# PaddlePaddle/MetaGym

Hardware: AMD Instinct MI355X
Metric: env-steps/sec (whole node) at 2^16 parallel envs; 1/2/4/8-GPU scaling (higher is better)
Workload: dtype f32/f64 mixed (reference choreography)

## Files before the change

metagym_amd/csrc/quadrotor.hip:

```cpp
#include <cstdlib>

#include "mg_common.h"
#include "mg_philox.h"

namespace {

#ifndef MG_QUAD_BLOCK
#define MG_QUAD_BLOCK 256
#endif
constexpr int BLOCK = MG_QUAD_BLOCK;
constexpr int WAVES_PER_BLOCK = BLOCK / mg::WAVE;
constexpr int OBS_DIM = 16;

struct QuadK {
    float phi32, phi_over_ra32, inv_jm32, mm32, prec32, ct0_32, ct1_32;
    float quality32, dt32, zoff32, healthy32, fail_range_sq32;
    float lm[4];
    float pc[12];
    float iinv[9];
    float df[9], dm[9];
    float cog[3];
    double prec, half_dt2, half_dt, ct2, quality, inv_quality;
    double min_v, max_v, fail_velocity, fail_w, healthy, xoff, yoff;
    int quality_recip_exact;
    int times, nt, task;
    int auto_reset;
    float init_v_base[3], init_w_base[3];
    double init_v_noisy, init_w_noisy;
    uint64_t seed, env_id_base;
    const int32_t *map;
    int map_h, map_w;
    const float *vtargets;
    int obs_dim;
};

struct Lane {
    float p[3];
    double v[3];
    double w[3];
    float pw[4];
    float R[9];
    double Rd[9];
    float Ri[9];
    double nv, nw;
    float power;
};


__device__ __forceinline__ double dot_row_f32f64(const float *row, const double *x) {
    return fma((double)row[2], x[2], fma((double)row[0], x[0], (double)row[1] * x[1]));
}

__device__ __forceinline__ void mv_f32f64(const float *M, const double *x, double *y) {
#pragma unroll
    for (int r = 0; r < 3; ++r) y[r] = dot_row_f32f64(&M[3 * r], x);
}

__device__ __forceinline__ void mv_f32(const float *M, const float *x, float *y) {
#pragma unroll
    for (int r = 0; r < 2; ++r) y[r] = (M[3 * r] * x[0] + M[3 * r + 1] * x[1]) + M[3 * r + 2] * x[2];
    y[2] = fmaf(M[8], x[2], fmaf(M[6], x[0], M[7] * x[1]));
}

__device__ __forceinline__ void mm_f32(const float *A, const float *B, float *C) {
#pragma unroll
    for (int r = 0; r < 3; ++r)
#pragma unroll
        for (int c = 0; c < 3; ++c)
            C[3 * r + c] = fmaf(A[3 * r + 2], B[6 + c], fmaf(A[3 * r + 1], B[3 + c], A[3 * r] * B[c]));
}

__device__ __forceinline__ void cross_f32(const float *a, const float *b, float *c) {
    float t0 = a[1] * b[2], t1 = a[2] * b[1];
    float t2 = a[2] * b[0], t3 = a[0] * b[2];
    float t4 = a[0] * b[1], t5 = a[1] * b[0];
    c[0] = t0 - t1;
    c[1] = t2 - t3;
    c[2] = t4 - t5;
}

__device__ __forceinline__ double norm3(const double *x) {
    return sqrt(fma(x[2], x[2], fma(x[1], x[1], x[0] * x[0])));
}
__device__ __forceinline__ float sumsq3(const float *x) {
    const float p0 = x[0] * x[0], p1 = x[1] * x[1], p2 = x[2] * x[2];
    return (float)(((double)p0 + (double)p1) + (double)p2);
}

__device__ __forceinline__ void inv3(const float *Af, float *Ainv, double *A) {
#pragma unroll
    for (int i = 0; i < 9; ++i) A[i] = (double)Af[i];
    const double c00 = fma(A[4], A[8], -(A[5] * A[7]));
    const double c01 = fma(A[5], A[6], -(A[3] * A[8]));
    const double c02 = fma(A[3], A[7], -(A[4] * A[6]));
    const double det = fma(A[2], c02, fma(A[1], c01, A[0] * c00));
    const double r = 1.0 / det;
    Ainv[0] = (float)(c00 * r);
    Ainv[3] = (float)(c01 * r);
    Ainv[6] = (float)(c02 * r);
    Ainv[1] = (float)(fma(A[2], A[7], -(A[1] * A[8])) * r);
    Ainv[4] = (float)(fma(A[0], A[8], -(A[2] * A[6])) * r);
    Ainv[7] = (float)(fma(A[1], A[6], -(A[0] * A[7])) * r);
    Ainv[2] = (float)(fma(A[1], A[5], -(A[2] * A[4])) * r);
    Ainv[5] = (float)(fma(A[2], A[3], -(A[0] * A[5])) * r);
    Ainv[8] = (float)(fma(A[0], A[4], -(A[1] * A[3])) * r);
}

template <bool SIMPLE, bool RECIP = false, bool XF = false>
__device__ __forceinline__ void substep(const QuadK &k, Lane &s, const float *eff32, bool want_power) {
    static_assert(!XF || SIMPLE, "the X frame is a SIMPLE configuration");
    float prop_force_z = 0.0f;
    float prop_torque[3] = {0.0f, 0.0f, 0.0f};
    float me[4], pp[4];

    const double bvz = dot_row_f32f64(&s.Ri[6], s.v);
    double xcz[4];
    if (XF) {
        const double c = (double)k.pc[1];
        const double A = s.w[0] * c, B = s.w[1] * c;
        xcz[0] = A - B;
        xcz[1] = A + B;
        xcz[2] = B - A;
        xcz[3] = (-A) - B;
    }

#pragma unroll
    for (int i = 0; i < 4; ++i) {
        const float e32 = eff32[i];
        float phi_w = k.phi32 * s.pw[i];
        me[i] = k.phi_over_ra32 * (e32 - phi_w);
        if (want_power) pp[i] = fabsf(me[i] / k.phi32 * e32);
        float d_prop_w = k.inv_jm32 * (me[i] - k.mm32);
        float w_m = s.pw[i] + k.prec32 * d_prop_w;
        const float *pc = &k.pc[3 * i];
        double cz = XF ? xcz[i] : s.w[0] * (double)pc[1] - s.w[1] * (double)pc[0];
        double v_1 = bvz + cz * (double)(XF ? k.lm[0] : k.lm[i]);
        float t0 = (k.ct0_32 * w_m) * w_m;
        double t1 = (double)(k.ct1_32 * w_m) * v_1;
        double thrust = (double)t0 + t1;
        if (!SIMPLE) {
            double sign = v_1 > 0 ? 1.0 : -1.0;
            thrust = thrust + ((k.ct2 * v_1) * v_1) * sign;
        }
        s.pw[i] = w_m;
        prop_force_z = (float)((double)prop_force_z + thrust);
        const float T = (float)thrust;
        if (XF) {
            const float Tc = T * k.pc[1];
            prop_torque[0] = (i < 2) ? prop_torque[0] + Tc : prop_torque[0] - Tc;
            prop_torque[1] = (i == 1 || i == 2) ? prop_torque[1] + Tc : prop_torque[1] - Tc;
        } else if (SIMPLE) {
            prop_torque[0] += T * pc[1];
            prop_torque[1] += (-T) * pc[0];
        } else {
            float a[3] = {-0.0f, -0.0f, -T};
            float cr[3];
            cross_f32(a, pc, cr);
            prop_torque[0] += cr[0];
            prop_torque[1] += cr[1];
            prop_torque[2] += cr[2];
        }
    }
    prop_torque[2] += ((-me[0] + me[1]) - me[2]) + me[3];

    float DfRi[9];
    double tmp[3], f_drag[3], t_drag[3];
    if (SIMPLE) {
#pragma unroll
        for (int r = 0; r < 3; ++r)
#pragma unroll
            for (int c = 0; c < 3; ++c) DfRi[3 * r + c] = k.df[4 * r] * s.Ri[3 * r + c];
    } else {
        mm_f32(k.df, s.Ri, DfRi);
    }
    mv_f32f64(DfRi, s.v, tmp);
    const double mnv = -s.nv;
#pragma unroll
    for (int c = 0; c < 3; ++c) f_drag[c] = mnv * tmp[c];
    if (SIMPLE) {
#pragma unroll
        for (int c = 0; c < 3; ++c) tmp[c] = (double)k.dm[4 * c] * s.w[c];
    } else {
        mv_f32f64(k.dm, s.w, tmp);
    }
    const double mnw = -s.nw;
#pragma unroll
    for (int c = 0; c < 3; ++c) t_drag[c] = mnw * tmp[c];

    float f_grav[3];
#pragma unroll
    for (int c = 0; c < 3; ++c) f_grav[c] = (s.Ri[3 * c + 2] * -9.8f) * k.quality32;

    double t_all[3], body_acc[3], acc[3];
    float t_grav_neg[3] = {0.0f, 0.0f, 0.0f};
    if (!SIMPLE) {
        float t_grav[3];
        cross_f32(f_grav, k.cog, t_grav);
#pragma unroll
        for (int c = 0; c < 3; ++c) t_grav_neg[c] = -t_grav[c];
    }
#pragma unroll
    for (int c = 0; c < 3; ++c) {
        const float pf = (c == 2) ? prop_force_z : 0.0f;
        double f_all = (double)(pf + f_grav[c]) + f_drag[c];
        t_all[c] = (double)(SIMPLE ? prop_torque[c] : prop_torque[c] + t_grav_neg[c]) + t_drag[c];
        body_acc[c] = (RECIP || k.quality_recip_exact) ? f_all * k.inv_quality : f_all / k.quality;
    }
#pragma unroll
    for (int r = 0; r < 3; ++r)
        acc[r] = fma(s.Rd[3 * r + 2], body_acc[2], fma(s.Rd[3 * r], body_acc[0], s.Rd[3 * r + 1] * body_acc[1]));
#pragma unroll
    for (int c = 0; c < 3; ++c)
        s.p[c] = (float)((double)s.p[c] + (s.v[c] * k.prec + k.half_dt2 * acc[c]));
#pragma unroll
    for (int c = 0; c < 3; ++c) s.v[c] = s.v[c] + k.prec * acc[c];
    if (want_power) s.power = ((pp[0] + pp[1]) + pp[2]) + pp[3];

    double alpha[3], tw[3];
    if (SIMPLE) {
#pragma unroll
        for (int c = 0; c < 3; ++c) alpha[c] = (double)k.iinv[4 * c] * t_all[c];
    } else {
        mv_f32f64(k.iinv, t_all, alpha);
    }
#pragma unroll
    for (int c = 0; c < 3; ++c) tw[c] = s.w[c] + k.half_dt * alpha[c];
    const float s01 = (float)(-tw[2]), s02 = (float)(tw[1]);
    const float s10 = (float)(tw[2]), s12 = (float)(-tw[0]);
    const float s20 = (float)(-tw[1]), s21 = (float)(tw[0]);
#pragma unroll
    for (int r = 0; r < 3; ++r) {
        const float r0 = s.R[3 * r], r1 = s.R[3 * r + 1], r2 = s.R[3 * r + 2];
        const float rs0 = fmaf(r2, s20, fmaf(r1, s10, r0 * 0.0f));
        const float rs1 = fmaf(r2, s21, fmaf(r1, 0.0f, r0 * s01));
        const float rs2 = fmaf(r2, 0.0f, fmaf(r1, s12, r0 * s02));
        s.R[3 * r] = r0 + k.prec32 * rs0;
        s.R[3 * r + 1] = r1 + k.prec32 * rs1;
        s.R[3 * r + 2] = r2 + k.prec32 * rs2;
    }
#pragma unroll
    for (int c = 0; c < 3; ++c) s.w[c] = s.w[c] + k.prec * alpha[c];
    inv3(s.R, s.Ri, s.Rd);
    s.nv = norm3(s.v);
    s.nw = norm3(s.w);
}

__device__ __forceinline__ int failure_code(const QuadK &k, const Lane &s) {
    const int c3 = (s.nw > k.fail_w) ? 3 : 0;
    const int c2 = (s.nv > k.fail_velocity) ? 2 : c3;
    return (sumsq3(s.p) > k.fail_range_sq32) ? 1 : c2;
}

__device__ __forceinline__ void observe(const QuadK &k, const Lane &s, float *obs) {
    double b_v[3];
    float b_pos[3], imu[3];
    const float g[3] = {0.0f, 0.0f, -9.8f};
    mv_f32f64(s.Ri, s.v, b_v);
    mv_f32(s.Ri, s.p, b_pos);
    mv_f32(s.Ri, g, imu);
    float roll = atan2f(s.R[7], s.R[8]);
    float pitch = atan2f(-s.R[6], sqrtf(s.R[7] * s.R[7] + s.R[8] * s.R[8]));
    float yaw = atan2f(s.R[3], s.R[0]);
    obs[0] = (float)b_v[0]; obs[1] = (float)b_v[1]; obs[2] = (float)b_v[2];
    obs[3] = b_pos[0]; obs[4] = b_pos[1]; obs[5] = b_pos[2];
    obs[6] = 0.0f + imu[0]; obs[7] = 0.0f + imu[1]; obs[8] = 0.0f + imu[2];
    obs[9] = (float)s.w[0]; obs[10] = (float)s.w[1]; obs[11] = (float)s.w[2];
    obs[12] = pitch; obs[13] = roll; obs[14] = yaw;
    obs[15] = s.p[2] + k.zoff32;
}

__device__ __forceinline__ void py_slice(long a, long b, long len, long &lo, long &hi) {
    if (a < 0) { a += len; if (a < 0) a = 0; } else if (a > len) a = len;
    if (b < 0) { b += len; if (b < 0) b = 0; } else if (b > len) b = len;
    lo = a; hi = b;
}

__device__ __forceinline__ bool collision(const QuadK &k, const double *op, const double *np_) {
    long mn[3], mx[3];
#pragma unroll
    for (int i = 0; i < 3; ++i) {
        double lo = op[i] < np_[i] ? op[i] : np_[i];
        double hi = op[i] > np_[i] ? op[i] : np_[i];
        mn[i] = (long)floor(lo);
        mx[i] = (long)ceil(hi);
    }
    int any = 0;
    if (k.map != nullptr) {
        long y0, y1, x0, x1;
        py_slice(mn[1], mx[1] + 1, k.map_h, y0, y1);
        py_slice(mn[0], mx[0] + 1, k.map_w, x0, x1);
        for (long y = y0; y < y1; ++y)
            for (long x = x0; x < x1; ++x) any |= (k.map[y * k.map_w + x] != 0);
    }
    return (mn[2] < any) || (mx[2] < any);
}

struct Lane32 {
    float p[3], v[3], w[3], pw[4], R[9], Ri[9];
};

__device__ void substep_f32state(const QuadK &k, Lane32 &s, const float *eff32) {
    float prop_force_z = 0.0f, prop_torque[3] = {0.0f, 0.0f, 0.0f}, me[4];
    const float ct2_32 = (float)k.ct2;
    for (int i = 0; i < 4; ++i) {
        const float e32 = eff32[i];
        float phi_w = k.phi32 * s.pw[i];
        me[i] = k.phi_over_ra32 * (e32 - phi_w);
        float d_prop_w = k.inv_jm32 * (me[i] - k.mm32);
        float w_m = s.pw[i] + k.prec32 * d_prop_w;
        const float *pc = &k.pc[3 * i];
        float bv[3], cr[3];
        mv_f32(s.Ri, s.v, bv);
        cross_f32(s.w, pc, cr);
        float v_1 = bv[2] + cr[2] * k.lm[i];
        float sign = v_1 > 0 ? 1.0f : -1.0f;
        float thrust = ((k.ct0_32 * w_m) * w_m + (k.ct1_32 * w_m) * v_1) + ((ct2_32 * v_1) * v_1) * sign;
        s.pw[i] = w_m;
        prop_force_z = prop_force_z + thrust;
        float a[3] = {-0.0f, -0.0f, -thrust};
        cross_f32(a, pc, cr);
        prop_torque[0] += cr[0]; prop_torque[1] += cr[1]; prop_torque[2] += cr[2];
    }
    prop_torque[2] += ((-me[0] + me[1]) - me[2]) + me[3];
    float DfRi[9], tmp[3], f_drag[3], t_drag[3];
    mm_f32(k.df, s.Ri, DfRi);
    mv_f32(DfRi, s.v, tmp);
    const float nv = -sqrtf(sumsq3(s.v));
    for (int c = 0; c < 3; ++c) f_drag[c] = nv * tmp[c];
    mv_f32(k.dm, s.w, tmp);
    const float nw = -sqrtf(sumsq3(s.w));
    for (int c = 0; c < 3; ++c) t_drag[c] = nw * tmp[c];
    const float g[3] = {0.0f, 0.0f, -9.8f};
    float f_grav[3], t_grav[3], body_acc[3], t_all[3], acc[3];
    mv_f32(s.Ri, g, f_grav);
    for (int c = 0; c < 3; ++c) f_grav[c] = f_grav[c] * k.quality32;
    cross_f32(f_grav, k.cog, t_grav);
    for (int c = 0; c < 3; ++c) {
        const float pf = (c == 2) ? prop_force_z : 0.0f;
        const float f_all = (pf + f_grav[c]) + f_drag[c];
        t_all[c] = (prop_torque[c] + (-t_grav[c])) + t_drag[c];
        body_acc[c] = f_all / k.quality32;
    }
    mv_f32(s.R, body_acc, acc);
    const float half_dt2 = (float)k.half_dt2, half_dt = (float)k.half_dt;
    for (int c = 0; c < 3; ++c) s.p[c] = s.p[c] + (s.v[c] * k.prec32 + half_dt2 * acc[c]);
    for (int c = 0; c < 3; ++c) s.v[c] = s.v[c] + k.prec32 * acc[c];
    float alpha[3], tw[3];
    mv_f32(k.iinv, t_all, alpha);
    for (int c = 0; c < 3; ++c) tw[c] = s.w[c] + half_dt * alpha[c];
    float S[9] = {0.0f, -tw[2], tw[1], tw[2], 0.0f, -tw[0], -tw[1], tw[0], 0.0f};
    float RS[9];
    mm_f32(s.R, S, RS);
    for (int c = 0; c < 9; ++c) s.R[c] = s.R[c] + k.prec32 * RS[c];
    for (int c = 0; c < 3; ++c) s.w[c] = s.w[c] + k.prec32 * alpha[c];
    double Rd[9];
    inv3(s.R, s.Ri, Rd);
}

__global__ void quadrotor_targets_kernel(QuadK k, int nt, const float *actions, float *targets) {
    if (blockIdx.x != 0 || threadIdx.x != 0) return;
    Lane32 s;
    for (int c = 0; c < 3; ++c) { s.p[c] = 0.0f; s.v[c] = 0.0f; s.w[c] = 0.0f; }
    for (int c = 0; c < 4; ++c) s.pw[c] = 0.0f;
    for (int c = 0; c < 9; ++c) { s.R[c] = (c % 4 == 0) ? 1.0f : 0.0f; s.Ri[c] = s.R[c]; }
    for (int t = 0; t < nt; ++t) {
        float eff32[4];
        for (int i = 0; i < 4; ++i) {
            double d = (double)actions[4 * t + i];
            d = d > k.max_v ? k.max_v : (d < k.min_v ? k.min_v : d);
            eff32[i] = (float)d;
        }
        for (int it = 0; it < k.times; ++it) substep_f32state(k, s, eff32);
        targets[3 * t] = s.v[0]; targets[3 * t + 1] = s.v[1]; targets[3 * t + 2] = s.v[2];
    }
}


template <typename T> __device__ __forceinline__ void st_stream(T *p, T v) { __builtin_nontemporal_store(v, p); }
typedef float v4f __attribute__((ext_vector_type(4)));
typedef uint32_t v2u __attribute__((ext_vector_type(2)));
typedef uint32_t v4u __attribute__((ext_vector_type(4)));

constexpr int AUX_NT = 2;
__device__ __forceinline__ __amdgpu_buffer_rsrc_t rsrc_of(const void *base, uint32_t bytes) {
    return __builtin_amdgcn_make_buffer_rsrc(const_cast<void *>(base), (short)0, (int)bytes, 0x00020000);
}
template <typename T> __device__ __forceinline__ T buf_ld(__amdgpu_buffer_rsrc_t r, uint32_t vo, uint32_t so) {
    if constexpr (sizeof(T) == 4) return __builtin_bit_cast(T, __builtin_amdgcn_raw_buffer_load_b32(r, vo, so, 0));
    else if constexpr (sizeof(T) == 8) return __builtin_bit_cast(T, __builtin_amdgcn_raw_buffer_load_b64(r, vo, so, 0));
    else return __builtin_bit_cast(T, __builtin_amdgcn_raw_buffer_load_b128(r, vo, so, 0));
}
template <int AUX, typename T> __device__ __forceinline__ void buf_st(T v, __amdgpu_buffer_rsrc_t r, uint32_t vo, uint32_t so) {
    if constexpr (sizeof(T) == 1) __builtin_amdgcn_raw_buffer_store_b8(__builtin_bit_cast(uint8_t, v), r, vo, so, AUX);
    else if constexpr (sizeof(T) == 4) __builtin_amdgcn_raw_buffer_store_b32(__builtin_bit_cast(uint32_t, v), r, vo, so, AUX);
    else if constexpr (sizeof(T) == 8) __builtin_amdgcn_raw_buffer_store_b64(__builtin_bit_cast(v2u, v), r, vo, so, AUX);
    else __builtin_amdgcn_raw_buffer_store_b128(__builtin_bit_cast(v4u, v), r, vo, so, AUX);
}
template <bool BUF, typename T> __device__ __forceinline__ T ld_soa(const T *a, int comps, int n, int c, int e) {
    if (!BUF) return a[(size_t)c * n + e];
    return buf_ld<T>(rsrc_of(a, (uint32_t)comps * (uint32_t)n * sizeof(T)), (uint32_t)e * sizeof(T),
                     (uint32_t)c * (uint32_t)n * sizeof(T));
}
template <bool BUF, typename T> __device__ __forceinline__ void st_soa(T *a, int comps, int n, int c, int e, T v) {
    if (!BUF) return st_stream(&a[(size_t)c * n + e], v);
    buf_st<AUX_NT>(v, rsrc_of(a, (uint32_t)comps * (uint32_t)n * sizeof(T)), (uint32_t)e * sizeof(T),
                   (uint32_t)c * (uint32_t)n * sizeof(T));
}

template <bool ROT_FIRST = false, bool BUF = false>
__device__ __forceinline__ void load_state(const mg_quadrotor_state &st, int n, int e, Lane &s, int &ct) {
    if (ROT_FIRST) {
#pragma unroll
        for (int c = 0; c < 9; ++c) s.R[c] = ld_soa<BUF>(st.rot, 9, n, c, e);
    }
    if (!ROT_FIRST) {
#pragma unroll
        for (int c = 0; c < 3; ++c) s.p[c] = ld_soa<BUF>(st.pos, 3, n, c, e);
    }
#pragma unroll
    for (int c = 0; c < 3; ++c) s.v[c] = ld_soa<BUF>(st.vel, 3, n, c, e);
#pragma unroll
    for (int c = 0; c < 3; ++c) s.w[c] = ld_soa<BUF>(st.omega, 3, n, c, e);
    if (ROT_FIRST) {
#pragma unroll
        for (int c = 0; c < 3; ++c) s.p[c] = ld_soa<BUF>(st.pos, 3, n, c, e);
    }
#pragma unroll
    for (int c = 0; c < 4; ++c) s.pw[c] = ld_soa<BUF>(st.propw, 4, n, c, e);
    if (!ROT_FIRST) {
#pragma unroll
        for (int c = 0; c < 9; ++c) s.R[c] = ld_soa<BUF>(st.rot, 9, n, c, e);
    }
    ct = ld_soa<BUF>(st.ct, 1, n, 0, e);
}

__device__ __forceinline__ void derive_lane(Lane &s) {
    inv3(s.R, s.Ri, s.Rd);
    s.nv = norm3(s.v);
    s.nw = norm3(s.w);
    s.power = 0.0f;
}

template <bool BUF = false>
__device__ __forceinline__ void load_lane(const mg_quadrotor_state &st, int n, int e, Lane &s, int &ct) {
    load_state<false, BUF>(st, n, e, s, ct);
    derive_lane(s);
}

template <bool BUF = false>
__device__ __forceinline__ void store_lane(const mg_quadrotor_state &st, int n, int e, const Lane &s, int ct) {
#pragma unroll
    for (int c = 0; c < 3; ++c) st_soa<BUF>(st.pos, 3, n, c, e, s.p[c]);
#pragma unroll
    for (int c = 0; c < 3; ++c) st_soa<BUF>(st.vel, 3, n, c, e, s.v[c]);
#pragma unroll
    for (int c = 0; c < 3; ++c) st_soa<BUF>(st.omega, 3, n, c, e, s.w[c]);
#pragma unroll
    for (int c = 0; c < 4; ++c) st_soa<BUF>(st.propw, 4, n, c, e, s.pw[c]);
#pragma unroll
    for (int c = 0; c < 9; ++c) st_soa<BUF>(st.rot, 9, n, c, e, s.R[c]);
    st_soa<BUF>(st.ct, 1, n, 0, e, ct);
}

template <bool BUF = false>
__device__ __forceinline__ void store_obs_wave(float *tile, const float *obs, float *out, int n, int e, int obs_dim) {
    if (!BUF && obs_dim != OBS_DIM) {
        if (e < n)
            for (int c = 0; c < obs_dim; ++c) out[(size_t)e * obs_dim + c] = obs[c];
        return;
    }
    const int lane = threadIdx.x & (mg::WAVE - 1);
    const int wave_base = e - lane;
    const bool full = (wave_base + mg::WAVE) <= n;
    if (full) {
#pragma unroll
        for (int c = 0; c < OBS_DIM; ++c) tile[lane * (OBS_DIM + 1) + c] = obs[c];
        __builtin_amdgcn_wave_barrier();
        float4 *dst = reinterpret_cast<float4 *>(out + (size_t)wave_base * OBS_DIM);
        const __amdgpu_buffer_rsrc_t r = rsrc_of(out, (uint32_t)n * (OBS_DIM * 4));
#pragma unroll
        for (int j = 0; j < 4; ++j) {
            const int q = j * mg::WAVE + lane;
            const int row = q >> 2, col = (q & 3) * 4;
            const float *src = &tile[row * (OBS_DIM + 1) + col];
            const v4f v{src[0], src[1], src[2], src[3]};
            if (BUF) buf_st<AUX_NT>(v, r, (uint32_t)(wave_base * OBS_DIM + 4 * lane) * 4 + j * (mg::WAVE * 16), 0);
            else st_stream(reinterpret_cast<v4f *>(dst + q), v);
        }
        __builtin_amdgcn_wave_barrier();
    } else if (e < n) {
        float4 *dst = reinterpret_cast<float4 *>(out + (size_t)e * OBS_DIM);
        const __amdgpu_buffer_rsrc_t r = rsrc_of(out, (uint32_t)n * (OBS_DIM * 4));
#pragma unroll
        for (int j = 0; j < 4; ++j) {
            const v4f v{obs[4 * j], obs[4 * j + 1], obs[4 * j + 2], obs[4 * j + 3]};
            if (BUF) buf_st<0>(v, r, (uint32_t)e * (OBS_DIM * 4) + j * 16, 0);
            else dst[j] = make_float4(v.x, v.y, v.z, v.w);
        }
    }
}

struct ResetDraw {
    double v[3], w[3], nv, nw;
};

__device__ __forceinline__ ResetDraw reset_draw(const QuadK &k, int e, uint32_t episode) {
    uint32_t r[8];
    const uint64_t gid = k.env_id_base + (uint64_t)e;
#pragma unroll
    for (int b = 0; b < 2; ++b)
        philox4x32_10((uint32_t)gid, (uint32_t)(gid >> 32), episode, (uint32_t)b, (uint32_t)k.seed,
                      (uint32_t)(k.seed >> 32), &r[4 * b]);
    const double inv32 = 1.0 / 4294967296.0;
    ResetDraw d;
#pragma unroll
    for (int c = 0; c < 3; ++c) {
        const double sv = ((r[6] >> c) & 1u) ? 1.0 : -1.0;
        const double sw = ((r[6] >> (3 + c)) & 1u) ? 1.0 : -1.0;
        d.v[c] = (double)k.init_v_base[c] + (k.init_v_noisy * ((double)r[c] * inv32)) * sv;
        d.w[c] = (double)k.init_w_base[c] + (k.init_w_noisy * ((double)r[3 + c] * inv32)) * sw;
    }
    d.nv = norm3(d.v);
    d.nw = norm3(d.w);
    return d;
}

__device__ __forceinline__ void reset_apply(Lane &s, const ResetDraw &d) {
#pragma unroll
    for (int c = 0; c < 3; ++c) {
        s.p[c] = 0.0f;
        s.v[c] = d.v[c];
        s.w[c] = d.w[c];
    }
#pragma unroll
    for (int c = 0; c < 4; ++c) s.pw[c] = 0.0f;
#pragma unroll
    for (int c = 0; c < 9; ++c) {
        s.R[c] = (c % 4 == 0) ? 1.0f : 0.0f;
        s.Ri[c] = s.R[c];
        s.Rd[c] = (double)s.R[c];
    }
    s.nv = d.nv;
    s.nw = d.nw;
    s.power = 0.0f;
}


struct StepIO {
    const float *action;
    float *obs;
    float *reward;
    double *reward64;
    uint8_t *done;
    uint8_t *failed;
};

struct KArgs { QuadK k; mg_quadrotor_state st; StepIO io; int n; int n_steps; };
typedef const __attribute__((address_space(4))) KArgs KArgsC;
__device__ __forceinline__ KArgsC *kernargs_fresh() {
    KArgsC *p = (KArgsC *)__builtin_amdgcn_kernarg_segment_ptr();
    asm volatile("" : "+s"(p));
    return p;
}

enum StepForm { STEP_GENERIC = 0, STEP_STOCK = 1, STEP_STOCK_SHADOW = 2 };
constexpr int STOCK_TIMES = 10;
#ifndef MG_QUAD_SUBSTEP_UNROLL
#define MG_QUAD_SUBSTEP_UNROLL 9
#endif

template <bool SIMPLE, int FORM, bool XF = false, bool BUF = false>
__global__ __launch_bounds__(BLOCK) void quadrotor_step_kernel(QuadK k, mg_quadrotor_state st, StepIO io,
                                                               int n, int n_steps_arg) {
    constexpr bool STOCK = FORM != STEP_GENERIC;
    constexpr bool SHADOW = FORM == STEP_STOCK_SHADOW;
    static_assert(!STOCK || SIMPLE, "the stock forms are SIMPLE");
    static_assert(STOCK || !XF, "XF is an option of the stock forms");
    static_assert(SHADOW || !BUF, "BUF is an option of STEP_STOCK_SHADOW");
    const int n_steps = SHADOW ? 1 : n_steps_arg;
    __shared__ float tiles[WAVES_PER_BLOCK][mg::WAVE * (OBS_DIM + 1)];
    const int e = blockIdx.x * BLOCK + threadIdx.x;
    const bool live = e < n;
    const int el = live ? e : n - 1;
    float *tile = tiles[threadIdx.x / mg::WAVE];

    {
        const uint32_t *ka = (const uint32_t *)__builtin_amdgcn_kernarg_segment_ptr();
        uint32_t touch = 0;
#pragma unroll
        for (int line = 0; line < (int)((sizeof(QuadK) + sizeof(mg_quadrotor_state) + sizeof(StepIO) + 8 + 63) / 64); ++line)
            touch |= ka[line * 16];
        asm volatile("" ::"s"(touch));
    }
    float4 a_next;
    Lane s;
    int ct;
    uint32_t episode = 0;
    ResetDraw rd;
    if (SHADOW) {
        episode = ld_soa<BUF>(st.episode, 1, n, 0, el);
        a_next = ld_soa<BUF>(reinterpret_cast<const float4 *>(io.action), 1, n, 0, el);
        load_state<true, BUF>(st, n, el, s, ct);
        __builtin_amdgcn_sched_barrier(0);
        rd = reset_draw(k, el, episode);
#pragma unroll
        for (int c = 0; c < 3; ++c) asm volatile("" : "+v"(rd.v[c]), "+v"(rd.w[c]));
        asm volatile("" : "+v"(rd.nv), "+v"(rd.nw));
        __builtin_amdgcn_sched_barrier(0);
        derive_lane(s);
        __builtin_amdgcn_sched_barrier(0);
    } else {
        a_next = reinterpret_cast<const float4 *>(io.action)[el];
        __builtin_amdgcn_sched_barrier(0);
        if (STOCK || k.auto_reset) episode = st.episode[el];
        load_lane(st, n, el, s, ct);
    }
    const uint32_t episode_in = episode;
    __builtin_amdgcn_s_waitcnt(0x0F70);

    for (int t = 0; t < n_steps; ++t) {
        const size_t off = (size_t)t * n;
        const float4 a = a_next;
        if (t + 1 < n_steps)
            a_next = reinterpret_cast<const float4 *>(io.action)[off + n + el];
        const float av[4] = {a.x, a.y, a.z, a.w};
        float eff32[4];
#pragma unroll
        for (int i = 0; i < 4; ++i) {
            double d = (double)av[i];
            d = d > k.max_v ? k.max_v : (d < k.min_v ? k.min_v : d);
            eff32[i] = (float)d;
        }
        ct += 1;
        const double old_pos[3] = {(double)s.p[0] + k.xoff, (double)s.p[1] + k.yoff,
                                   (double)(s.p[2] + k.zoff32)};
        int fail = 0;
        if (STOCK) {
#pragma unroll MG_QUAD_SUBSTEP_UNROLL
            for (int it = 0; it < STOCK_TIMES - 1; ++it) {
                substep<SIMPLE, true, XF>(k, s, eff32, false);
                const int code = failure_code(k, s);
                fail = fail ? fail : code;
            }
            substep<SIMPLE, true, XF>(k, s, eff32, true);
            const int code = failure_code(k, s);
            fail = fail ? fail : code;
        } else {
            for (int it = 0; it < k.times; ++it) {
                if (fail == 0) {
                    substep<SIMPLE>(k, s, eff32, it == k.times - 1);
                    fail = failure_code(k, s);
                }
            }
        }
        const KArgsC *kae = kernargs_fresh();
        const QuadK &ke = *(const QuadK *)&kae->k;
        const StepIO &ioe = *(const StepIO *)&kae->io;
        const bool vel_task = ke.task == MG_QUADROTOR_TASK_VELOCITY_CONTROL;
        const int tn_step = ct < ke.nt - 1 ? ct : ke.nt - 1;
        double reward = 0.0;
        int done = 1;
        if (fail == 0 && vel_task) {
            float bt[3];
            mv_f32(s.Ri, &ke.vtargets[3 * (ct - 1)], bt);
            double b_v[3];
            mv_f32f64(s.Ri, s.v, b_v);
            const double diff = (fabs((double)bt[0] - b_v[0]) + fabs((double)bt[1] - b_v[1])) + fabs((double)bt[2] - b_v[2]);
            const float energy = ke.dt32 * s.power;
            const double r = (ke.healthy32 < energy) ? -ke.healthy : -(double)energy;
            reward = r + (-0.001 * diff);
            done = 0;
            if (ct == ke.nt) { done = 1; ct = 0; }
        } else if (fail == 0) {
            const double new_pos[3] = {(double)s.p[0] + ke.xoff, (double)s.p[1] + ke.yoff,
                                       (double)(s.p[2] + ke.zoff32)};
            const bool hit = collision(ke, old_pos, new_pos);
            const float energy = ke.dt32 * s.power;
            double r = (ke.healthy32 < energy) ? -ke.healthy : -(double)energy;
            double task_reward = hit ? 0.0 : ke.healthy;
            if (ke.task == MG_QUADROTOR_TASK_HOVERING_CONTROL) {
                task_reward -= 1.0 * s.nv + 1.0 * s.nw;
                const float z_move = fabsf(0.0f - s.p[2]);
                if (z_move < 0.5f) task_reward += 10;
                else {
                    const float o = 0.5f - z_move;
                    task_reward += (o > -20.0f) ? (double)o : -20.0;
                }
            }
            if (ke.task == MG_QUADROTOR_TASK_HOVERING_CONTROL || ke.healthy32 < energy)
                reward = r + task_reward;
            else
                reward = (double)((float)r + (float)task_reward);
            done = 0;
            if (hit) { done = 1; ct = 0; }
            if (ct == ke.nt) { done = 1; ct = 0; }
        } else {
            ct = 0;
        }
        int tn = tn_step;
        if ((STOCK || ke.auto_reset) && done) {
            if (SHADOW) reset_apply(s, rd);
            else reset_apply(s, reset_draw(ke, el, episode));
            episode += 1;
            tn = ct < ke.nt - 1 ? ct : ke.nt - 1;
        }
        if (t + 1 < n_steps) asm volatile("" : "+v"(a_next.x), "+v"(a_next.y), "+v"(a_next.z), "+v"(a_next.w));
        if (t == n_steps - 1 && live) {
            const mg_quadrotor_state &ste = *(const mg_quadrotor_state *)&kae->st;
            store_lane<BUF>(ste, n, e, s, ct);
            if (episode != episode_in) st_soa<BUF>(ste.episode, 1, n, 0, e, episode);
        }
        __builtin_amdgcn_sched_barrier(0);
        float obs[OBS_DIM + 3];
        observe(ke, s, obs);
        if (vel_task) { obs[16] = ke.vtargets[3 * tn]; obs[17] = ke.vtargets[3 * tn + 1]; obs[18] = ke.vtargets[3 * tn + 2]; }
        store_obs_wave<BUF>(tile, obs, ioe.obs + off * ke.obs_dim, n, e, ke.obs_dim);
        if (live) {
            if (BUF) {
                if (ioe.reward) st_soa<true>(ioe.reward + off, 1, n, 0, e, (float)reward);
                if (ioe.reward64) st_soa<true>(ioe.reward64 + off, 1, n, 0, e, reward);
                st_soa<true>(ioe.done + off, 1, n, 0, e, (uint8_t)done);
                if (ioe.failed) st_soa<true>(ioe.failed + off, 1, n, 0, e, (uint8_t)fail);
            } else {
                if (ioe.reward) st_stream(&ioe.reward[off + e], (float)reward);
                if (ioe.reward64) st_stream(&ioe.reward64[off + e], reward);
                st_stream(&ioe.done[off + e], (uint8_t)done);
                if (ioe.failed) st_stream(&ioe.failed[off + e], (uint8_t)fail);
            }
        }
    }
}

__global__ __launch_bounds__(BLOCK) void quadrotor_reset_kernel(QuadK k, mg_quadrotor_state st,
                                                                const uint8_t *mask, const double *init_vel,
                                                                const double *init_omega, float *obs_out, int n) {
    const int e = blockIdx.x * BLOCK + threadIdx.x;
    if (e >= n) return;
    if (mask != nullptr && mask[e] == 0) return;
    Lane s;
#pragma unroll
    for (int c = 0; c < 3; ++c) {
        s.p[c] = 0.0f;
        s.v[c] = init_vel ? init_vel[(size_t)c * n + e] : 0.0;
        s.w[c] = init_omega ? init_omega[(size_t)c * n + e] : 0.0;
    }
#pragma unroll
    for (int c = 0; c < 4; ++c) s.pw[c] = 0.0f;
#pragma unroll
    for (int c = 0; c < 9; ++c) s.R[c] = (c % 4 == 0) ? 1.0f : 0.0f;
    inv3(s.R, s.Ri, s.Rd);
    s.nv = norm3(s.v);
    s.nw = norm3(s.w);
    s.power = 0.0f;
    const int ct = st.ct[e];
    store_lane(st, n, e, s, ct);
    if (obs_out != nullptr) {
        float obs[OBS_DIM + 3];
        observe(k, s, obs);
        if (k.task == MG_QUADROTOR_TASK_VELOCITY_CONTROL) {
            const int tn = ct < k.nt - 1 ? ct : k.nt - 1;
            obs[16] = k.vtargets[3 * tn]; obs[17] = k.vtargets[3 * tn + 1]; obs[18] = k.vtargets[3 * tn + 2];
        }
        for (int c = 0; c < k.obs_dim; ++c) obs_out[(size_t)e * k.obs_dim + c] = obs[c];
    }
}


void host_inv3_f32(const float *Af, float *Ainv) {
    double A[9];
    for (int i = 0; i < 9; ++i) A[i] = (double)Af[i];
    const double c00 = fma(A[4], A[8], -(A[5] * A[7])), c01 = fma(A[5], A[6], -(A[3] * A[8])),
                 c02 = fma(A[3], A[7], -(A[4] * A[6]));
    const double det = fma(A[2], c02, fma(A[1], c01, A[0] * c00));
    const double r = 1.0 / det;
    Ainv[0] = (float)(c00 * r); Ainv[3] = (float)(c01 * r); Ainv[6] = (float)(c02 * r);
    Ainv[1] = (float)(fma(A[2], A[7], -(A[1] * A[8])) * r);
    Ainv[4] = (float)(fma(A[0], A[8], -(A[2] * A[6])) * r);
    Ainv[7] = (float)(fma(A[1], A[6], -(A[0] * A[7])) * r);
    Ainv[2] = (float)(fma(A[1], A[5], -(A[2] * A[4])) * r);
    Ainv[5] = (float)(fma(A[2], A[3], -(A[0] * A[5])) * r);
    Ainv[8] = (float)(fma(A[0], A[4], -(A[1] * A[3])) * r);
}

int fold_config(const mg_quadrotor_config *c, QuadK *k, bool need_targets = true) {
    if (!(c->precision >= 1e-8) || c->precision > c->dt)
        return mg::set_error(MG_ERR_BAD_CONFIG, "precision %g must be in [1e-8, dt=%g]", c->precision, c->dt);
    if (c->task != MG_QUADROTOR_TASK_NO_COLLISION && c->task != MG_QUADROTOR_TASK_HOVERING_CONTROL &&
        c->task != MG_QUADROTOR_TASK_VELOCITY_CONTROL)
        return mg::set_error(MG_ERR_UNSUPPORTED, "quadrotor task %d is not implemented", c->task);
    if (c->task == MG_QUADROTOR_TASK_VELOCITY_CONTROL && need_targets && c->velocity_targets_d == nullptr)
        return mg::set_error(MG_ERR_NULL_POINTER, "velocity_control needs cfg->velocity_targets_d");
    if (c->map_d != nullptr && (c->map_h <= 0 || c->map_w <= 0))
        return mg::set_error(MG_ERR_BAD_SIZE, "map shape %d x %d", c->map_h, c->map_w);
    k->phi32 = (float)c->phi;
    k->phi_over_ra32 = (float)(c->phi / c->ra);
    k->inv_jm32 = (float)(1.0 / c->jm);
    k->mm32 = (float)c->mm;
    k->prec32 = (float)c->precision;
    k->ct0_32 = (float)c->ct0;
    k->ct1_32 = (float)c->ct1;
    k->quality32 = (float)c->quality;
    k->dt32 = (float)c->dt;
    k->zoff32 = (float)c->z_offset;
    k->healthy32 = (float)c->healthy_reward;
    {
        const float T = (float)c->fail_range;
        float S;
        if (T < 0.0f) {
            S = -INFINITY;
        } else if (T == INFINITY) {
            S = INFINITY;
        } else {
            S = T * T;
            while (sqrtf(S) > T) S = nextafterf(S, 0.0f);
            while (sqrtf(nextafterf(S, INFINITY)) <= T) S = nextafterf(S, INFINITY);
        }
        k->fail_range_sq32 = S;
    }
    for (int i = 0; i < 4; ++i) {
        const float *p = &c->prop_coord[3 * i];
        const float p0 = p[0] * p[0], p1 = p[1] * p[1], p2 = p[2] * p[2];
        k->lm[i] = sqrtf((float)(((double)p0 + (double)p1) + (double)p2));
    }
    for (int i = 0; i < 12; ++i) k->pc[i] = c->prop_coord[i];
    host_inv3_f32(c->inertia, k->iinv);
    for (int i = 0; i < 9; ++i) { k->df[i] = c->drag_f[i]; k->dm[i] = c->drag_m[i]; }
    for (int i = 0; i < 3; ++i) k->cog[i] = c->gravity_center[i];
    k->prec = c->precision;
    k->half_dt2 = 0.5 * c->precision * c->precision;
    k->half_dt = 0.5 * c->precision;
    k->ct2 = c->ct2;
    k->quality = c->quality;
    k->inv_quality = 1.0 / c->quality;
    int ex = 0;
    (void)frexp(c->quality, &ex);
    k->quality_recip_exact = (frexp(c->quality, &ex) == 0.5) ? 1 : 0;
    k->min_v = c->min_voltage;
    k->max_v = c->max_voltage;
    k->fail_velocity = c->fail_velocity;
    k->fail_w = c->fail_w;
    k->healthy = c->healthy_reward;
    k->xoff = (double)c->x_offset;
    k->yoff = (double)c->y_offset;
    k->times = (int)(c->dt / c->precision);
    k->nt = c->nt;
    k->task = c->task;
    k->map = c->map_d;
    k->map_h = c->map_h;
    k->map_w = c->map_w;
    k->vtargets = c->velocity_targets_d;
    k->obs_dim = c->task == MG_QUADROTOR_TASK_VELOCITY_CONTROL ? 19 : 16;
    k->auto_reset = 0;
    for (int i = 0; i < 3; ++i) { k->init_v_base[i] = 0.0f; k->init_w_base[i] = 0.0f; }
    k->init_v_noisy = k->init_w_noisy = 0.0;
    k->seed = k->env_id_base = 0;
    return MG_OK;
}

bool config_is_simple(const mg_quadrotor_config *c) {
    for (int r = 0; r < 3; ++r)
        for (int col = 0; col < 3; ++col)
            if (r != col && (c->drag_f[3 * r + col] != 0.0f || c->drag_m[3 * r + col] != 0.0f ||
                             c->inertia[3 * r + col] != 0.0f))
                return false;
    for (int i = 0; i < 3; ++i)
        if (c->gravity_center[i] != 0.0f) return false;
    for (int i = 0; i < 4; ++i)
        if (c->prop_coord[3 * i + 2] != 0.0f) return false;
    return c->ct2 == 0.0;
}

bool config_is_xframe(const mg_quadrotor_config *cfg) {
    const float *pc = cfg->prop_coord;
    const float c = pc[1];
    const float sx[4] = {1.0f, -1.0f, -1.0f, 1.0f}, sy[4] = {1.0f, 1.0f, -1.0f, -1.0f};
    if (!(c > 0.0f && c < INFINITY)) return false;
    for (int i = 0; i < 4; ++i)
        if (pc[3 * i] != sx[i] * c || pc[3 * i + 1] != sy[i] * c || pc[3 * i + 2] != 0.0f) return false;
    return true;
}

int check_state(const mg_quadrotor_state *s) {
    if (!s->pos || !s->vel || !s->omega || !s->propw || !s->rot || !s->ct)
        return mg::set_error(MG_ERR_NULL_POINTER, "mg_quadrotor_state has a NULL array");
    return MG_OK;
}

struct Plan {
    uint32_t magic;
    int32_t n, device, simple;
    int32_t stock;
    int32_t xframe;
    int32_t simds;
    QuadK k;
    mg_quadrotor_state st;
};
constexpr uint32_t PLAN_MAGIC = 0x4d475150u;
static_assert(sizeof(Plan) <= sizeof(mg_quadrotor_plan), "mg_quadrotor_plan is too small for the folded constants");

int make_plan(Plan *p, const mg_quadrotor_config *cfg, const mg_quadrotor_autoreset *ar, int32_t n,
              const mg_quadrotor_state *state) {
    MG_REQUIRE_PTR(cfg);
    MG_REQUIRE_PTR(state);
    if (n <= 0) return mg::set_error(MG_ERR_BAD_SIZE, "n_envs=%d", n);
    if (int rc = check_state(state)) return rc;
    if (int rc = fold_config(cfg, &p->k)) return rc;
    if (ar != nullptr) {
        if (state->episode == nullptr)
            return mg::set_error(MG_ERR_NULL_POINTER, "fused auto-reset needs mg_quadrotor_state.episode");
        QuadK &k = p->k;
        k.auto_reset = 1;
        for (int i = 0; i < 3; ++i) { k.init_v_base[i] = ar->init_velocity[i]; k.init_w_base[i] = ar->init_angular_velocity[i]; }
        k.init_v_noisy = ar->init_velocity_noisy;
        k.init_w_noisy = ar->init_angular_velocity_noisy;
        k.seed = ar->seed;
        k.env_id_base = ar->env_id_base;
    }
    p->magic = PLAN_MAGIC;
    p->n = n;
    p->device = mg::device_of(state->pos);
    p->simple = (config_is_simple(cfg) && cfg->task != MG_QUADROTOR_TASK_VELOCITY_CONTROL) ? 1 : 0;
    const bool force_generic = getenv("MG_QUAD_GENERIC") != nullptr;
    p->stock = (!force_generic && p->simple && p->k.quality_recip_exact && p->k.times == STOCK_TIMES && p->k.auto_reset) ? 1 : 0;
    p->xframe = (p->stock && config_is_xframe(cfg)) ? 1 : 0;
    p->simds = 0;
    int cus = 0;
    if (p->device >= 0 && hipDeviceGetAttribute(&cus, hipDeviceAttributeMultiprocessorCount, p->device) == hipSuccess)
        p->simds = 4 * cus;
    else
        (void)hipGetLastError();
    p->st = *state;
    return MG_OK;
}

int launch_plan(const Plan *p, int32_t n_steps, const float *action, float *obs, float *reward, double *reward64,
                uint8_t *done, uint8_t *failed, void *stream) {
    MG_REQUIRE_PTR(action);
    MG_REQUIRE_PTR(obs);
    MG_REQUIRE_PTR(done);
    if (n_steps <= 0) return mg::set_error(MG_ERR_BAD_SIZE, "n_steps=%d", n_steps);
    mg::DeviceGuard guard(p->device);
    StepIO io{action, obs, reward, reward64, done, failed};
    const int n = p->n, grid = (n + BLOCK - 1) / BLOCK;
    const int waves = (n + mg::WAVE - 1) / mg::WAVE;
    const bool buf = (uint64_t)n * (OBS_DIM * sizeof(float)) < (1ull << 31);
    constexpr int SH = STEP_STOCK_SHADOW;
    decltype(&quadrotor_step_kernel<false, STEP_GENERIC>) kern;
    if (p->stock && n_steps == 1 && waves <= p->simds) {
        if (p->xframe) kern = buf ? quadrotor_step_kernel<true, SH, true, true> : quadrotor_step_kernel<true, SH, true, false>;
        else kern = buf ? quadrotor_step_kernel<true, SH, false, true> : quadrotor_step_kernel<true, SH, false, false>;
    } else if (p->stock) {
        kern = p->xframe ? quadrotor_step_kernel<true, STEP_STOCK, true> : quadrotor_step_kernel<true, STEP_STOCK>;
    } else if (p->simple) {
        kern = quadrotor_step_kernel<true, STEP_GENERIC>;
    } else {
        kern = quadrotor_step_kernel<false, STEP_GENERIC>;
    }
    hipLaunchKernelGGL(kern, dim3(grid), dim3(BLOCK), 0, (hipStream_t)stream, p->k, p->st, io, n, n_steps);
    return mg::check_launch("quadrotor_step_kernel");
}

int launch_steps(const mg_quadrotor_config *cfg, int32_t n, int32_t n_steps, const mg_quadrotor_state *state,
                 const float *action, float *obs, float *reward, double *reward64, uint8_t *done,
                 uint8_t *failed, void *stream, const mg_quadrotor_autoreset *ar = nullptr) {
    MG_REQUIRE_PTR(cfg);
    MG_REQUIRE_PTR(state);
    MG_REQUIRE_PTR(action);
    MG_REQUIRE_PTR(obs);
    MG_REQUIRE_PTR(done);
    Plan p;
    if (int rc = make_plan(&p, cfg, ar, n, state)) return rc;
    return launch_plan(&p, n_steps, action, obs, reward, reward64, done, failed, stream);
}

}

extern "C" int mg_quadrotor_default_config(mg_quadrotor_config *c) {
    MG_REQUIRE_PTR(c);
    *c = mg_quadrotor_config{};
    c->precision = 0.001;
    c->quality = 0.5;
    c->ct0 = 1.538e-5; c->ct1 = -2.5e-4; c->ct2 = 0.0;
    c->mm = 0.010; c->jm = 2.573e-4; c->ra = 0.2010; c->phi = 0.017242179827506;
    c->fail_velocity = 100.0; c->fail_w = 1000.0; c->fail_range = 1000.0;
    c->min_voltage = 0.10; c->max_voltage = 15.0;
    c->dt = 0.01; c->healthy_reward = 1.0; c->z_offset = 5.0;
    c->x_offset = 50; c->y_offset = 50;
    c->nt = 1000;
    c->task = MG_QUADROTOR_TASK_NO_COLLISION;
    c->inertia[0] = 0.0135f; c->inertia[4] = 0.0135f; c->inertia[8] = 0.024f;
    c->drag_m[0] = 0.074f; c->drag_m[4] = 0.074f; c->drag_m[8] = 0.0506f;
    c->drag_f[0] = 0.12f; c->drag_f[4] = 0.12f; c->drag_f[8] = 0.10f;
    const float pc[12] = {0.18f, 0.18f, 0.f, -0.18f, 0.18f, 0.f, -0.18f, -0.18f, 0.f, 0.18f, -0.18f, 0.f};
    for (int i = 0; i < 12; ++i) c->prop_coord[i] = pc[i];
    c->map_d = nullptr; c->map_h = 100; c->map_w = 100;
    return MG_OK;
}

extern "C" int mg_quadrotor_velocity_targets(const mg_quadrotor_config *cfg, int32_t nt, const float *actions_d,
                                             float *targets_d, void *stream) {
    MG_REQUIRE_PTR(cfg);
    MG_REQUIRE_PTR(actions_d);
    MG_REQUIRE_PTR(targets_d);
    if (nt <= 0) return mg::set_error(MG_ERR_BAD_SIZE, "nt=%d", nt);
    QuadK k;
    if (int rc = fold_config(cfg, &k, false)) return rc;
    mg::DeviceGuard guard(mg::device_of(targets_d));
    hipLaunchKernelGGL(quadrotor_targets_kernel, dim3(1), dim3(64), 0, (hipStream_t)stream, k, nt, actions_d, targets_d);
    return mg::check_launch("quadrotor_targets_kernel");
}

extern "C" int mg_quadrotor_reset(const mg_quadrotor_config *cfg, int32_t n, const mg_quadrotor_state *state,
                                  const uint8_t *mask, const double *init_vel, const double *init_omega,
                                  float *obs, void *stream) {
    MG_REQUIRE_PTR(cfg);
    MG_REQUIRE_PTR(state);
    if (n <= 0) return mg::set_error(MG_ERR_BAD_SIZE, "n_envs=%d", n);
    if (int rc = check_state(state)) return rc;
    QuadK k;
    if (int rc = fold_config(cfg, &k)) return rc;
    const int grid = (n + BLOCK - 1) / BLOCK;
    mg::DeviceGuard guard(mg::device_of(state->pos));
    hipLaunchKernelGGL(quadrotor_reset_kernel, dim3(grid), dim3(BLOCK), 0, (hipStream_t)stream, k, *state, mask,
                       init_vel, init_omega, obs, n);
    return mg::check_launch("quadrotor_reset_kernel");
}

extern "C" int mg_quadrotor_step(const mg_quadrotor_config *cfg, int32_t n, const mg_quadrotor_state *state,
                                 const float *action, float *obs, float *reward, double *reward64,
                                 uint8_t *done, uint8_t *failed, void *stream) {
    return launch_steps(cfg, n, 1, state, action, obs, reward, reward64, done, failed, stream);
}

extern "C" int mg_quadrotor_step_autoreset(const mg_quadrotor_config *cfg, int32_t n, int32_t n_steps,
                                           const mg_quadrotor_state *state, const mg_quadrotor_autoreset *ar,
                                           const float *action, float *obs, float *reward, double *reward64,
                                           uint8_t *done, uint8_t *failed, void *stream) {
    MG_REQUIRE_PTR(ar);
    return launch_steps(cfg, n, n_steps, state, action, obs, reward, reward64, done, failed, stream, ar);
}

extern "C" int mg_quadrotor_rollout(const mg_quadrotor_config *cfg, int32_t n, int32_t n_steps,
                                    const mg_quadrotor_state *state, const float *action, float *obs,
                                    float *reward, double *reward64, uint8_t *done, uint8_t *failed,
                                    void *stream) {
    return launch_steps(cfg, n, n_steps, state, action, obs, reward, reward64, done, failed, stream);
}

extern "C" int mg_quadrotor_plan_init(mg_quadrotor_plan *plan, const mg_quadrotor_config *cfg,
                                      const mg_quadrotor_autoreset *ar, int32_t n_envs,
                                      const mg_quadrotor_state *state) {
    MG_REQUIRE_PTR(plan);
    Plan *p = reinterpret_cast<Plan *>(plan);
    p->magic = 0;
    return make_plan(p, cfg, ar, n_envs, state);
}

extern "C" int mg_quadrotor_plan_step(const mg_quadrotor_plan *plan, int32_t n_steps, const float *action, float *obs,
                                      float *reward, double *reward64, uint8_t *done, uint8_t *failed, void *stream) {
    MG_REQUIRE_PTR(plan);
    const Plan *p = reinterpret_cast<const Plan *>(plan);
    if (p->magic != PLAN_MAGIC) return mg::set_error(MG_ERR_BAD_CONFIG, "mg_quadrotor_plan is not initialised");
    return launch_plan(p, n_steps, action, obs, reward, reward64, done, failed, stream);
}
```

Measured before the change: 4.618 billion.

## Replace f64 divide and sqrt with Newton-refined hardware approximations plus guarded fallback

In the shadow stock step kernel, the per-substep 3x3 inverse determinant reciprocal and the two velocity norms now use the hardware rcp/rsq approximations refined by Newton iterations, instead of full IEEE f64 division and sqrt. An exponent-range check flags inputs where the refinement might not match exactly. If any lane in the wave is flagged, the wave reloads its state and recomputes the step on the exact path. The aim is to drop the costly f64 div/sqrt sequences from the hot loop, at the cost of extra registers, a ballot per step and a rare slow fallback. Optional phase timestamp instrumentation is also added behind a macro.

```diff
diff --git a/metagym_amd/csrc/quadrotor.hip b/metagym_amd/csrc/quadrotor.hip
--- a/metagym_amd/csrc/quadrotor.hip
+++ b/metagym_amd/csrc/quadrotor.hip
@@ -79,25 +79,55 @@
     c[2] = t4 - t5;
 }
 
-__device__ __forceinline__ double norm3(const double *x) {
-    return sqrt(fma(x[2], x[2], fma(x[1], x[1], x[0] * x[0])));
+__device__ __forceinline__ double sumsq3(const double *x) {
+    return fma(x[2], x[2], fma(x[1], x[1], x[0] * x[0]));
+}
+__device__ __forceinline__ double norm3(const double *x) { return sqrt(sumsq3(x)); }
+
+__device__ __forceinline__ uint32_t hi_word(double x) { return (uint32_t)(__builtin_bit_cast(uint64_t, x) >> 32); }
+__device__ __forceinline__ bool all_in_range(double xv, double xw, double d) {
+    constexpr uint32_t SPAN = 1000u << 20, SQRT_BASE = 256u << 20, RCP_BASE = 523u << 20;
+    const uint32_t tv = xv == 0.0 ? 0u : hi_word(xv) - SQRT_BASE, tw = xw == 0.0 ? 0u : hi_word(xw) - SQRT_BASE;
+    const uint32_t td = (hi_word(d) & 0x7fffffffu) - RCP_BASE;
+    return max(tv, max(tw, td)) < SPAN;
+}
+__device__ __forceinline__ double sqrt_newton(double x) {
+    const double g = fmin(__builtin_amdgcn_rsq(x), 0x1p+512);
+    double s = x * g, h = g * 0.5;
+    const double r = fma(-h, s, 0.5);
+    s = fma(s, r, s);
+    h = fma(h, r, h);
+    const double d0 = fma(-s, s, x);
+    s = fma(d0, h, s);
+    const double d1 = fma(-s, s, x);
+    return fma(d1, h, s);
+}
+__device__ __forceinline__ double rcp_newton(double d) {
+    double y = __builtin_amdgcn_rcp(d);
+    y = fma(y, fma(-d, y, 1.0), y);
+    y = fma(y, fma(-d, y, 1.0), y);
+    return fma(fma(-d, y, 1.0), y, y);
 }
 __device__ __forceinline__ float sumsq3(const float *x) {
     const float p0 = x[0] * x[0], p1 = x[1] * x[1], p2 = x[2] * x[2];
     return (float)(((double)p0 + (double)p1) + (double)p2);
 }
 
-__device__ __forceinline__ void inv3(const float *Af, float *Ainv, double *A) {
+struct Cof { double c00, c01, c02, det; };
+__device__ __forceinline__ Cof inv3_cof(const float *Af, double *A) {
 #pragma unroll
     for (int i = 0; i < 9; ++i) A[i] = (double)Af[i];
-    const double c00 = fma(A[4], A[8], -(A[5] * A[7]));
-    const double c01 = fma(A[5], A[6], -(A[3] * A[8]));
-    const double c02 = fma(A[3], A[7], -(A[4] * A[6]));
-    const double det = fma(A[2], c02, fma(A[1], c01, A[0] * c00));
-    const double r = 1.0 / det;
-    Ainv[0] = (float)(c00 * r);
-    Ainv[3] = (float)(c01 * r);
-    Ainv[6] = (float)(c02 * r);
+    Cof c;
+    c.c00 = fma(A[4], A[8], -(A[5] * A[7]));
+    c.c01 = fma(A[5], A[6], -(A[3] * A[8]));
+    c.c02 = fma(A[3], A[7], -(A[4] * A[6]));
+    c.det = fma(A[2], c.c02, fma(A[1], c.c01, A[0] * c.c00));
+    return c;
+}
+__device__ __forceinline__ void inv3_scale(const double *A, const Cof &c, double r, float *Ainv) {
+    Ainv[0] = (float)(c.c00 * r);
+    Ainv[3] = (float)(c.c01 * r);
+    Ainv[6] = (float)(c.c02 * r);
     Ainv[1] = (float)(fma(A[2], A[7], -(A[1] * A[8])) * r);
     Ainv[4] = (float)(fma(A[0], A[8], -(A[2] * A[6])) * r);
     Ainv[7] = (float)(fma(A[1], A[6], -(A[0] * A[7])) * r);
@@ -105,9 +135,30 @@
     Ainv[5] = (float)(fma(A[2], A[3], -(A[0] * A[5])) * r);
     Ainv[8] = (float)(fma(A[0], A[4], -(A[1] * A[3])) * r);
 }
-
-template <bool SIMPLE, bool RECIP = false, bool XF = false>
-__device__ __forceinline__ void substep(const QuadK &k, Lane &s, const float *eff32, bool want_power) {
+__device__ __forceinline__ void inv3(const float *Af, float *Ainv, double *A) {
+    const Cof c = inv3_cof(Af, A);
+    inv3_scale(A, c, 1.0 / c.det, Ainv);
+}
+
+template <bool FAST>
+__device__ __forceinline__ void update_derived(Lane &s, bool &ok) {
+    if (!FAST) {
+        inv3(s.R, s.Ri, s.Rd);
+        s.nv = norm3(s.v);
+        s.nw = norm3(s.w);
+        return;
+    }
+    const Cof c = inv3_cof(s.R, s.Rd);
+    const double xv = sumsq3(s.v), xw = sumsq3(s.w);
+    const double r = rcp_newton(c.det), nv = sqrt_newton(xv), nw = sqrt_newton(xw);
+    ok = ok & all_in_range(xv, xw, c.det);
+    inv3_scale(s.Rd, c, r, s.Ri);
+    s.nv = nv;
+    s.nw = nw;
+}
+
+template <bool SIMPLE, bool RECIP = false, bool XF = false, bool FAST = false>
+__device__ __forceinline__ void substep(const QuadK &k, Lane &s, const float *eff32, bool want_power, bool &ok) {
     static_assert(!XF || SIMPLE, "the X frame is a SIMPLE configuration");
     float prop_force_z = 0.0f;
     float prop_torque[3] = {0.0f, 0.0f, 0.0f};
@@ -240,9 +291,7 @@
     }
 #pragma unroll
     for (int c = 0; c < 3; ++c) s.w[c] = s.w[c] + k.prec * alpha[c];
-    inv3(s.R, s.Ri, s.Rd);
-    s.nv = norm3(s.v);
-    s.nw = norm3(s.w);
+    update_derived<FAST>(s, ok);
 }
 
 __device__ __forceinline__ int failure_code(const QuadK &k, const Lane &s) {
@@ -434,17 +483,17 @@
     ct = ld_soa<BUF>(st.ct, 1, n, 0, e);
 }
 
-__device__ __forceinline__ void derive_lane(Lane &s) {
-    inv3(s.R, s.Ri, s.Rd);
-    s.nv = norm3(s.v);
-    s.nw = norm3(s.w);
+template <bool FAST = false>
+__device__ __forceinline__ void derive_lane(Lane &s, bool &ok) {
+    update_derived<FAST>(s, ok);
     s.power = 0.0f;
 }
 
 template <bool BUF = false>
 __device__ __forceinline__ void load_lane(const mg_quadrotor_state &st, int n, int e, Lane &s, int &ct) {
+    bool ok = true;
     load_state<false, BUF>(st, n, e, s, ct);
-    derive_lane(s);
+    derive_lane<false>(s, ok);
 }
 
 template <bool BUF = false>
@@ -564,7 +613,27 @@
 }
 
 enum StepForm { STEP_GENERIC = 0, STEP_STOCK = 1, STEP_STOCK_SHADOW = 2 };
+
+#ifdef MG_QUAD_PHASE_STAMPS
+constexpr int PHASE_STAMPS = 5, PHASE_SLOTS = 8, PHASE_MAX_WAVES = 4096;
+__device__ uint64_t g_phase_stamps[PHASE_MAX_WAVES * PHASE_SLOTS];
+#define MG_PHASE_STAMP(i)                                                                 \
+    do {                                                                                  \
+        if (SHADOW) {                                                                     \
+            __builtin_amdgcn_sched_barrier(0);                                            \
+            stamp[i] = __builtin_amdgcn_s_memrealtime();                                  \
+            __builtin_amdgcn_sched_barrier(0);                                            \
+        }                                                                                 \
+    } while (0)
+#else
+#define MG_PHASE_STAMP(i) \
+    do {                  \
+    } while (0)
+#endif
 constexpr int STOCK_TIMES = 10;
+#ifndef MG_QUAD_FASTPATH
+#define MG_QUAD_FASTPATH 1
+#endif
 #ifndef MG_QUAD_SUBSTEP_UNROLL
 #define MG_QUAD_SUBSTEP_UNROLL 9
 #endif
@@ -577,6 +646,7 @@
     static_assert(!STOCK || SIMPLE, "the stock forms are SIMPLE");
     static_assert(STOCK || !XF, "XF is an option of the stock forms");
     static_assert(SHADOW || !BUF, "BUF is an option of STEP_STOCK_SHADOW");
+    constexpr bool FAST = SHADOW && MG_QUAD_FASTPATH;
     const int n_steps = SHADOW ? 1 : n_steps_arg;
     __shared__ float tiles[WAVES_PER_BLOCK][mg::WAVE * (OBS_DIM + 1)];
     const int e = blockIdx.x * BLOCK + threadIdx.x;
@@ -592,6 +662,13 @@
             touch |= ka[line * 16];
         asm volatile("" ::"s"(touch));
     }
+#ifdef MG_QUAD_PHASE_STAMPS
+    uint64_t stamp[PHASE_STAMPS];
+    uint32_t fallbacks = 0;
+    const uint64_t clock_in = __builtin_readcyclecounter();
+#endif
+    MG_PHASE_STAMP(0);
+    bool ok = true;
     float4 a_next;
     Lane s;
     int ct;
@@ -607,7 +684,7 @@
         for (int c = 0; c < 3; ++c) asm volatile("" : "+v"(rd.v[c]), "+v"(rd.w[c]));
         asm volatile("" : "+v"(rd.nv), "+v"(rd.nw));
         __builtin_amdgcn_sched_barrier(0);
-        derive_lane(s);
+        derive_lane<false>(s, ok);
         __builtin_amdgcn_sched_barrier(0);
     } else {
         a_next = reinterpret_cast<const float4 *>(io.action)[el];
@@ -617,6 +694,7 @@
     }
     const uint32_t episode_in = episode;
     __builtin_amdgcn_s_waitcnt(0x0F70);
+    MG_PHASE_STAMP(1);
 
     for (int t = 0; t < n_steps; ++t) {
         const size_t off = (size_t)t * n;
@@ -638,21 +716,39 @@
         if (STOCK) {
 #pragma unroll MG_QUAD_SUBSTEP_UNROLL
             for (int it = 0; it < STOCK_TIMES - 1; ++it) {
-                substep<SIMPLE, true, XF>(k, s, eff32, false);
+                substep<SIMPLE, true, XF, FAST>(k, s, eff32, false, ok);
                 const int code = failure_code(k, s);
                 fail = fail ? fail : code;
             }
-            substep<SIMPLE, true, XF>(k, s, eff32, true);
+            substep<SIMPLE, true, XF, FAST>(k, s, eff32, true, ok);
             const int code = failure_code(k, s);
             fail = fail ? fail : code;
+            if (FAST && __builtin_expect(__builtin_amdgcn_ballot_w64(!ok) != 0, 0)) {
+                const KArgsC *kaf = kernargs_fresh();
+                const QuadK &kf = *(const QuadK *)&kaf->k;
+                int ct_loaded;
+                load_state<true, BUF>(*(const mg_quadrotor_state *)&kaf->st, n, el, s, ct_loaded);
+                derive_lane<false>(s, ok);
+                fail = 0;
+#pragma unroll 1
+                for (int it = 0; it < STOCK_TIMES; ++it) {
+                    substep<SIMPLE, true, XF, false>(kf, s, eff32, it == STOCK_TIMES - 1, ok);
+                    const int code = failure_code(kf, s);
+                    fail = fail ? fail : code;
+                }
+#ifdef MG_QUAD_PHASE_STAMPS
+                fallbacks += 1;
+#endif
+            }
         } else {
             for (int it = 0; it < k.times; ++it) {
                 if (fail == 0) {
-                    substep<SIMPLE>(k, s, eff32, it == k.times - 1);
+                    substep<SIMPLE>(k, s, eff32, it == k.times - 1, ok);
                     fail = failure_code(k, s);
                 }
             }
         }
+        MG_PHASE_STAMP(2);
         const KArgsC *kae = kernargs_fresh();
         const QuadK &ke = *(const QuadK *)&kae->k;
         const StepIO &ioe = *(const StepIO *)&kae->io;
@@ -710,11 +806,13 @@
             store_lane<BUF>(ste, n, e, s, ct);
             if (episode != episode_in) st_soa<BUF>(ste.episode, 1, n, 0, e, episode);
         }
+        MG_PHASE_STAMP(3);
         __builtin_amdgcn_sched_barrier(0);
         float obs[OBS_DIM + 3];
         observe(ke, s, obs);
         if (vel_task) { obs[16] = ke.vtargets[3 * tn]; obs[17] = ke.vtargets[3 * tn + 1]; obs[18] = ke.vtargets[3 * tn + 2]; }
         store_obs_wave<BUF>(tile, obs, ioe.obs + off * ke.obs_dim, n, e, ke.obs_dim);
+        MG_PHASE_STAMP(4);
         if (live) {
             if (BUF) {
                 if (ioe.reward) st_soa<true>(ioe.reward + off, 1, n, 0, e, (float)reward);
@@ -729,6 +827,20 @@
             }
         }
     }
+#ifdef MG_QUAD_PHASE_STAMPS
+    if (SHADOW) {
+        const uint32_t wave = (blockIdx.x * BLOCK + threadIdx.x) / mg::WAVE;
+        if ((threadIdx.x & (mg::WAVE - 1)) == 0 && wave < PHASE_MAX_WAVES) {
+            uint64_t *out = &g_phase_stamps[(size_t)wave * PHASE_SLOTS];
+#pragma unroll
+            for (int i = 0; i < PHASE_STAMPS; ++i) out[i] = stamp[i];
+            out[5] = clock_in;
+            out[6] = (uint64_t)__builtin_amdgcn_s_getreg((31 << 11) | 4) |
+                     ((uint64_t)__builtin_amdgcn_s_getreg((31 << 11) | 20) << 32);
+            out[7] = (uint64_t)fallbacks << 32;
+        }
+    }
+#endif
 }
 
 __global__ __launch_bounds__(BLOCK) void quadrotor_reset_kernel(QuadK k, mg_quadrotor_state st,
@@ -1056,6 +1168,16 @@
     return make_plan(p, cfg, ar, n_envs, state);
 }
 
+#ifdef MG_QUAD_PHASE_STAMPS
+extern "C" int mg_quadrotor_phase_stamps(uint64_t *host, int32_t max_waves) {
+    MG_REQUIRE_PTR(host);
+    const int32_t w = max_waves < PHASE_MAX_WAVES ? max_waves : PHASE_MAX_WAVES;
+    if (hipMemcpyFromSymbol(host, HIP_SYMBOL(g_phase_stamps), (size_t)w * PHASE_SLOTS * sizeof(uint64_t)) != hipSuccess)
+        return mg::set_error(MG_ERR_UNSUPPORTED, "hipMemcpyFromSymbol(g_phase_stamps) failed");
+    return MG_OK;
+}
+#endif
+
 extern "C" int mg_quadrotor_plan_step(const mg_quadrotor_plan *plan, int32_t n_steps, const float *action, float *obs,
                                       float *reward, double *reward64, uint8_t *done, uint8_t *failed, void *stream) {
     MG_REQUIRE_PTR(plan);
```

Result: faster. 4.797 billion, median of 6 (+3.9%).
